# Malfoy/Brisk

Hardware: AMD Instinct MI355X
Metric: distinct k-mers indexed/sec (k=63,m=21) (higher is better)
Workload: dtype u64; 1 GPU; 1x MI355X: 50M synthetic 150 bp reads per GPU, k=63 m=21 b=14, uint8 counts, 15x coverage; reads_per_gpu=50000000, total_reads=50000000, part_bits=24, genome_len=500000000, parallelism=single GPU

## Files before the change

brisk_amd/csrc/brisk_capi.hip:

```cpp
#include "brisk_kernels.hip"

#include <algorithm>
#include <atomic>
#include <cerrno>
#include <chrono>
#include <cmath>
#include <cstdio>
#include <cstdlib>
#include <cstring>
#include <mutex>
#include <new>
#include <string>
#include <thread>
#include <vector>

#include <fcntl.h>
#include <sys/stat.h>
#include <unistd.h>

#include "../../include/brisk_hip.h"

#if !defined(__HIP_DEVICE_COMPILE__) && defined(__x86_64__)
#include <immintrin.h>
#define BRISK_HOST_AVX2 1
// ... 34 lines not shown
    u32 n_rerun, pad;
    unsigned long long kept;
    unsigned long long n_ovf;
    unsigned long long slice_sum;
    u32 upsert_done, pad2;
    struct Result { unsigned long long w[3]; } result;
    unsigned long long dbg_guard;
};
static_assert(sizeof(Counters::Scan) == sizeof(unsigned long long) + 2 * sizeof(u32) && sizeof(Counters::Touched) == 2 * sizeof(u32) + sizeof(unsigned long long), "ScanOut; k_touched, k_need");
static_assert(sizeof(Counters::Kmers) == 2 * sizeof(unsigned long long) && sizeof(Counters::Result) == 3 * sizeof(unsigned long long), "k_count_kmers: out[0..1]; k_checksum: out[0..2]");
static_assert(sizeof(Counters::Work) == 6 * sizeof(u32) && sizeof(Counters::Plan) == 2 * sizeof(u32), "32-bit counters throughout");
struct PinnedCounters : Counters {
    u32 n_huge;
    unsigned long long arena_used;
    unsigned long long n_rec_new;
    unsigned long long prof[3];
    unsigned long long answers;
};

}

struct brisk_hip_index {
    BriskParams P{};
    int device = 0;
    hipStream_t stream = nullptr;
    bool own_stream = false;
    std::string err;
    std::recursive_mutex call_mu;
    u64 n_parts = 0, n_buckets = 0;
    u64 max_batch_reads = 0;

    double* d_coef = nullptr;
    double* d_tabs = nullptr;
    ScanCfg scfg{};
    u32 dbg_touched_last = 0;
    u64 dbg_guard_last = 0;
    bool fresh = true;
    u32 insert_waves = 4096;
    u32 scan_waves = 0;
    size_t scan_lds = 0;
    bool scan_v1 = false;
    bool entry_ids = false;
    u32 count_mode = 0;
    bool use_vmm = false;
    bool scan_hist_valid = false;
    u64 arena_limit = 0;
    VmBuf vm_keys, vm_counts, vm_ids;
    unsigned long long* d_id_counter = nullptr;
    DevBuf seq_buf;
    u64 arena_cap = 0;
    u64 arena_used_host = 0;
    IndexDev ix{};
    DevBuf route_buf;
    DevBuf bins;
    DevBuf left;
    DevBuf huge;
    DevBuf pend;
    u64 n_pend = 0;
    bool pend_hist_ok = true;
    bool defer = true;
    bool verify = false;
    bool trace = false;
    DevBuf staging, parted, desc, chunk_buf, tags_a, tags_b, packed_tmp, bases_tmp, starts_tmp, sums_tmp, enum_out, lookup_buf;
    DevBuf packed_tmp2, starts_tmp2;
    DevBuf anchors, slot_buf, kout_tmp;
    DevBuf prof_out, prof_plan;
// ... 546 lines not shown
                HIPCHK(h, fetch_ctr_sync(h, &h->d_ctr->work));
                fprintf(stderr, "[brisk_hip] k_insert_first: %u of %u partitions taken in pairs, %u table-free, %u left over\n", h->h_ctr->work.n_pair, n_touched,
                        h->h_ctr->work.n_clean, h->h_ctr->work.n_left);
            }
        }
        if (n_huge) {
            if (sat) hipLaunchKernelGGL(k_insert_huge<true>, dim3(std::min<u32>(n_huge, 256u)), dim3(HG_THREADS), 0, h->stream, P, src, (const PartDesc*)h->desc.p,
                                        (const u32*)h->huge.p + 1, (const u32*)h->huge.p, h->ix);
            else hipLaunchKernelGGL(k_insert_huge<false>, dim3(std::min<u32>(n_huge, 256u)), dim3(HG_THREADS), 0, h->stream, P, src, (const PartDesc*)h->desc.p,
                                    (const u32*)h->huge.p + 1, (const u32*)h->huge.p, h->ix);
            if ((rc = launch_check(h, "k_insert_huge"))) return rc;
        }
    }
    h->nb_skmers += n_rec;
    h->dir_snapshot_valid = false;
    return BRISK_HIP_OK;
}

int launch_scan(brisk_hip_index* h, const u32* d_packed, const u64* d_starts, u64 n_items, const ScanOut& out, bool query_mode, bool plain,
                const ChunkCtl& cc, bool pos = false) {
    ProfScope ps(h, S_SCAN);
    if (plain && !pos) {
        BriskParams P = h->P;
        if (out.ret) {
            P.ext_bits -= P.cls_bits;
            P.cls_bits = 0;
        }
        hipLaunchKernelGGL(k_scan, dim3(nblocks(n_items, SCAN_BLOCK)), dim3(SCAN_BLOCK), 0, h->stream, P, d_packed, d_starts, n_items, h->d_coef,
                           out, query_mode ? 1 : 0);
    } else {
        const u32 bt = h->scan_waves * 64;
        const dim3 grid(nblocks(n_items, bt)), block(bt);
#define LAUNCH_SCAN2(NCH, MODE, KK, MM) \
    hipLaunchKernelGGL((k_scan2<NCH, MODE, KK, MM>), grid, block, h->scan_lds - scan_fixed_tabs(MM) * 8, h->stream, ScanArgs{h->P, h->scfg, d_packed, d_starts, n_items, h->d_tabs, out, cc})
#define LAUNCH_SCAN2_MODES(NCH, KK, MM)                    \
    {                                                      \
        if (pos && cc.vreads) LAUNCH_SCAN2(NCH, 4, KK, MM);  \
        else if (pos) LAUNCH_SCAN2(NCH, 3, KK, MM);        \
        else if (cc.vreads) LAUNCH_SCAN2(NCH, 2, KK, MM);  \
        else if (query_mode) LAUNCH_SCAN2(NCH, 1, KK, MM); \
        else LAUNCH_SCAN2(NCH, 0, KK, MM);                 \
    }
        const u32 k = h->P.k, m = h->P.m;
        if (k == 63 && m == 21) LAUNCH_SCAN2_MODES(0, 63, 21)
        else if (k == 31 && m == 15) LAUNCH_SCAN2_MODES(0, 31, 15)
        else if (k == 31 && m == 11) LAUNCH_SCAN2_MODES(0, 31, 11)
        else if (h->scfg.nch == 6) LAUNCH_SCAN2_MODES(6, 0, 0)
        else if (h->scfg.nch == 4) LAUNCH_SCAN2_MODES(4, 0, 0)
        else if (h->scfg.nch == 3) LAUNCH_SCAN2_MODES(3, 0, 0)
        else LAUNCH_SCAN2_MODES(0, 0, 0)
#undef LAUNCH_SCAN2_MODES
#undef LAUNCH_SCAN2
    }
    return launch_check(h, "k_scan");
}

enum class ScanMode { Insert, Query, Sequence, Position };
struct ScanReq {
    ScanMode mode;
    const u32* d_packed; const u64* d_starts; u64 n_reads;
    u64* d_rec; u64 cap;
    u64 kmer_bound = 0;
    bool with_hist = false, keep_hist = false;
    u32* d_tags = nullptr;
    u64* d_side = nullptr;
    const u64* d_slot_base = nullptr;
};
// ... 836 lines not shown
            return rc;
        }
    }
    if (h->profiling) {
        h->prof_ms[S_UPLOAD] += up_ms;
        h->prof_launches[S_UPLOAD] += subs.size();
    }
    return BRISK_HIP_OK;
}

int drain_profile(brisk_hip_index* h) {
    if (h->pending.empty()) return BRISK_HIP_OK;
    HIPCHK(h, hipStreamSynchronize(h->stream));
    for (auto& pe : h->pending) {
        float ms = 0;
        hipEventElapsedTime(&ms, pe.a, pe.b);
        h->prof_ms[pe.slot] += ms;
        h->prof_launches[pe.slot]++;
        hipEventDestroy(pe.a);
        hipEventDestroy(pe.b);
    }
    h->pending.clear();
    return BRISK_HIP_OK;
}

void free_all(brisk_hip_index* h) {
    hipStreamSynchronize(h->stream);
    auto fr = [](void* p) { if (p) hipFree(p); };
    for (DevBuf* b : {&h->huge, &h->left, &h->pend, &h->bins, &h->staging, &h->parted, &h->desc, &h->chunk_buf, &h->route_buf, &h->tags_a, &h->tags_b, &h->packed_tmp, &h->bases_tmp, &h->starts_tmp, &h->sums_tmp, &h->enum_out,
                      &h->lookup_buf, &h->packed_tmp2, &h->starts_tmp2, &h->anchors, &h->slot_buf, &h->kout_tmp, &h->prof_out, &h->prof_plan, &h->reck_buf, &h->ext_iv, &h->ext_tmp, &h->ext_src, &h->ink_mask, &h->ink_tmp, &h->ink_tab, &h->ink_raw, &h->ink_offs, &h->ink_packed, &h->pair_tab, &h->pair_iv, &h->pair_raw, &h->pair_fs, &h->split_off, &h->split_tab, &h->corr_sites, &h->corr_rows, &h->corr_cand, &h->corr_slots, &h->corr_tmp, &h->corr_tab})
        fr(b->p);
    fr(h->d_coef);
    fr(h->d_tabs);
    if (h->use_vmm) {
        pool_give(h->device, h->vm_keys, h->vm_counts, h->vm_ids);
    } else {
        fr(h->ix.keys);
        fr(h->ix.counts);
        fr(h->ix.ids);
    }
    fr(h->d_id_counter);
    fr(h->ix.err);
    fr(h->seq_buf.p);
    fr(h->ix.dir);
    fr(h->ix.cursor);
    fr(h->ix.bucket_bits);
    fr(h->ix.stats);
    fr(h->ix.slot_cur);
    fr(h->ix.slot_end);
    fr(h->d_hist);
    fr(h->d_ovf_cnt);
    fr(h->d_owner_cut);
    fr(h->d_off);
    fr(h->d_cur32);
    fr(h->d_touched);
    fr(h->d_block_sums);
    fr(h->d_ctr);
    if (h->h_ctr) hipHostFree(h->h_ctr);
    if (h->h_pin) hipHostFree(h->h_pin);
    for (auto& pe : h->pending) {
        hipEventDestroy(pe.a);
        hipEventDestroy(pe.b);
    }
    if (h->own_stream && h->stream) hipStreamDestroy(h->stream);
}

// ... 78 lines not shown
        HIPCHK(h, hipMalloc((void**)&h->d_coef, 128 * sizeof(double)));
        HIPCHK(h, hipMemsetAsync(h->d_coef, 0, 128 * sizeof(double), h->stream));
        HIPCHK(h, hipMemcpyAsync(h->d_coef, coef_table, 4 * m * sizeof(double), hipMemcpyHostToDevice, h->stream));
        {
            ScanCfg& c = h->scfg;
            c.nlow = std::min<u32>(32, k);
            c.nlow1 = std::min<u32>(32, k - 1);
            c.nch = cls_nch(m);
            c.qcap = 320;
            if (c.nch > CLS_MAX_CHUNKS) return fail(h, BRISK_HIP_EUNSUPPORTED, "minimizer too long for the class tables");
            const u32 n_tab = 128 + cls_base(m, c.nch);
            c.n_tab = n_tab;
            std::vector<double> tabs(n_tab, 0.0);
            for (u32 i = 0; i < 4u * m; i++) tabs[i] = coef_table[i];
            for (u32 ch = 0; ch < c.nch; ch++) {
                const u32 off = cls_off(m, ch), wd = cls_width(m, ch), base = cls_base(m, ch);
                c.chunk[ch] = (2 * off) | ((2 * wd) << 6) | (base << 10);
                for (u32 v = 0; v < (1u << (2 * wd)); v++) {
                    double a = 0.0, bsum = 0.0;
                    for (u32 i = off; i < off + wd; i++) {
                        const u32 nt = (v >> (2 * (i - off))) & 3;
                        if (i + 1 < m) a += coef_table[4 * (m - 1 - i) + nt];
                        if (i >= 1) bsum += coef_table[4 * (m - i) + nt];
                    }
                    const int64_t af = llround(std::ldexp(a, 24)), bf = llround(std::ldexp(bsum, 24));
                    u64 word = (u64)af + ((u64)bf << 32);
                    if (ch == 0) word += ((u64)CLS_BIAS << 32) + CLS_BIAS;
                    memcpy(&tabs[128 + base + v], &word, 8);
                }
            }
            HIPCHK(h, hipMalloc((void**)&h->d_tabs, n_tab * sizeof(double)));
            HIPCHK(h, hipMemcpyAsync(h->d_tabs, tabs.data(), n_tab * sizeof(double), hipMemcpyHostToDevice, h->stream));
            HIPCHK(h, hipStreamSynchronize(h->stream));
            const size_t fixed = (size_t)(n_tab + 9) * 8;
            const size_t lds_max = 160 * 1024;
            const bool spec = (k == 63 && m == 21) || (k == 31 && m == 15) || (k == 31 && m == 11);
            u32 blocks_per_cu = std::max<u32>(1, (u32)(scan_waves_per_eu(spec ? (int)k : 0, spec ? (int)m : 0) * 4) / 8);
            auto lds_of = [&](u32 q, u32 waves) { return fixed + waves * (size_t)(q + 96) * 8; };
            while (blocks_per_cu > 1 && blocks_per_cu * lds_of(224, 8) > lds_max - 2048) blocks_per_cu--;
            while (c.qcap > 224 && blocks_per_cu * lds_of(c.qcap, 8) > lds_max - 2048) c.qcap -= 32;
            if (const char* e = getenv("BRISK_SCAN_QCAP")) c.qcap = (u32)std::max(128, atoi(e));
            const size_t per_wave = (size_t)(c.qcap + 96) * 8;
            u32 wv = 8;
            if (lds_of(c.qcap, 8) > lds_max) wv = (u32)std::min<size_t>(16, (lds_max - fixed) / per_wave);
            if (const char* e = getenv("BRISK_SCAN_WAVES")) wv = (u32)std::min(16, std::max(1, atoi(e)));
            h->scan_waves = wv;
            h->scan_lds = fixed + wv * per_wave;
            static size_t lds_attr = 0;
            if (h->scan_lds > lds_attr) {
                lds_attr = h->scan_lds;
                struct FnLds { const void* fn; size_t fixed; };
#define SCAN2_FNS(NCH, KK, MM) FnLds{(const void*)k_scan2<NCH, 0, KK, MM>, scan_fixed_tabs(MM) * 8}, FnLds{(const void*)k_scan2<NCH, 1, KK, MM>, scan_fixed_tabs(MM) * 8}, \
                               FnLds{(const void*)k_scan2<NCH, 2, KK, MM>, scan_fixed_tabs(MM) * 8}, FnLds{(const void*)k_scan2<NCH, 3, KK, MM>, scan_fixed_tabs(MM) * 8}, \
                               FnLds{(const void*)k_scan2<NCH, 4, KK, MM>, scan_fixed_tabs(MM) * 8}
#define DEBUG_FN(NCH, MM) FnLds{(const void*)k_debug_keys<NCH, MM>, scan_fixed_tabs(MM) * 8}
                const FnLds fns[] = {SCAN2_FNS(0, 0, 0), SCAN2_FNS(3, 0, 0), SCAN2_FNS(4, 0, 0), SCAN2_FNS(6, 0, 0), SCAN2_FNS(0, 31, 11), SCAN2_FNS(0, 31, 15), SCAN2_FNS(0, 63, 21),
                                     DEBUG_FN(0, 0), DEBUG_FN(3, 0), DEBUG_FN(4, 0), DEBUG_FN(6, 0), DEBUG_FN(0, 11), DEBUG_FN(0, 15), DEBUG_FN(0, 21)};
#undef DEBUG_FN
#undef SCAN2_FNS
                for (const FnLds& f : fns) HIPCHK(h, hipFuncSetAttribute(f.fn, hipFuncAttributeMaxDynamicSharedMemorySize, (int)std::min(lds_attr, lds_max - f.fixed)));
            }
            const char* v1 = getenv("BRISK_SCAN_V1");
            h->scan_v1 = v1 && v1[0] == '1';
        }
        {
            const void* fns[] = {(const void*)k_insert<0, 0, 0>, (const void*)k_insert_big<0, 0, 0>, (const void*)k_insert_fast<3, 49, 4>, (const void*)k_insert_first<3, 49, 4>, (const void*)k_insert_fast<2, 17, 4>,
// ... 1770 lines not shown
    return launch_check(h, "k_synth");
}

BRISK_API int brisk_hip_debug_order_keys(brisk_hip_index* h, const uint64_t* mmers, uint64_t n, int exact, uint64_t* keys) {
    if (!h || (n && (!mmers || !keys))) return BRISK_HIP_EINVAL;
    if (!n) return BRISK_HIP_OK;
    HIPCHK(h, hipSetDevice(h->device));
    std::lock_guard<std::recursive_mutex> call_lock(h->call_mu);
    int rc;
    if ((rc = ensure(h, h->lookup_buf, n * 16))) return rc;
    u64* d_x = (u64*)h->lookup_buf.p;
    u64* d_k = d_x + n;
    HIPCHK(h, hipMemcpyAsync(d_x, mmers, n * 8, hipMemcpyHostToDevice, h->stream));
    const size_t lds = (size_t)h->scfg.n_tab * 8;
    HIPCHK(h, zero_ctr(h, &h->d_ctr->dbg_guard));
#define LAUNCH_DEBUG_KEYS(NCH, MM) \
    hipLaunchKernelGGL((k_debug_keys<NCH, MM>), dim3(nblocks(n, 256)), dim3(256), lds - scan_fixed_tabs(MM) * 8, h->stream, h->P, h->scfg, h->d_tabs, d_x, n, exact, d_k, &h->d_ctr->dbg_guard)
    const u32 k = h->P.k, m = h->P.m;
    if (k == 63 && m == 21) LAUNCH_DEBUG_KEYS(0, 21);
    else if (k == 31 && m == 15) LAUNCH_DEBUG_KEYS(0, 15);
    else if (k == 31 && m == 11) LAUNCH_DEBUG_KEYS(0, 11);
    else if (h->scfg.nch == 6) LAUNCH_DEBUG_KEYS(6, 0);
    else if (h->scfg.nch == 4) LAUNCH_DEBUG_KEYS(4, 0);
    else if (h->scfg.nch == 3) LAUNCH_DEBUG_KEYS(3, 0);
    else LAUNCH_DEBUG_KEYS(0, 0);
#undef LAUNCH_DEBUG_KEYS
    if ((rc = launch_check(h, "k_debug_keys"))) return rc;
    HIPCHK(h, hipMemcpyAsync(keys, d_k, n * 8, hipMemcpyDeviceToHost, h->stream));
    HIPCHK(h, fetch_ctr_sync(h, &h->d_ctr->dbg_guard));
    h->dbg_guard_last = h->h_ctr->dbg_guard;
    return BRISK_HIP_OK;
}

BRISK_API int brisk_hip_debug_guard_count(brisk_hip_index* h, uint64_t* n_guard) {
    if (!h || !n_guard) return BRISK_HIP_EINVAL;
    std::lock_guard<std::recursive_mutex> call_lock(h->call_mu);
    *n_guard = h->dbg_guard_last;
    return BRISK_HIP_OK;
}

BRISK_API int brisk_hip_debug_touched(brisk_hip_index* h, uint32_t* parts, uint64_t cap, uint64_t* n) {
    if (!h || !n || (cap && !parts)) return BRISK_HIP_EINVAL;
    HIPCHK(h, hipSetDevice(h->device));
    std::lock_guard<std::recursive_mutex> call_lock(h->call_mu);
    *n = h->dbg_touched_last;
    const u64 take = std::min<u64>(cap, h->dbg_touched_last);
    if (take) HIPCHK(h, hipMemcpyAsync(parts, h->d_touched, take * 4, hipMemcpyDeviceToHost, h->stream));
    HIPCHK(h, hipStreamSynchronize(h->stream));
    return BRISK_HIP_OK;
}

BRISK_API int brisk_hip_debug_directory(brisk_hip_index* h, const uint32_t* parts, uint64_t n, uint32_t* cnt, uint32_t* cap) {
    if (!h || (n && (!parts || !cnt || !cap))) return BRISK_HIP_EINVAL;
    HIPCHK(h, hipSetDevice(h->device));
    std::lock_guard<std::recursive_mutex> call_lock(h->call_mu);
    for (u64 i = 0; i < n; i++)
        if (parts[i] >= h->n_parts) return BRISK_HIP_EINVAL;
    std::vector<DirEnt> dir(h->n_parts);
    HIPCHK(h, hipMemcpyAsync(dir.data(), h->ix.dir, h->n_parts * sizeof(DirEnt), hipMemcpyDeviceToHost, h->stream));
    HIPCHK(h, hipStreamSynchronize(h->stream));
    for (u64 i = 0; i < n; i++) {
        cnt[i] = dir[parts[i]].cnt;
        cap[i] = dir[parts[i]].cap;
    }
    return BRISK_HIP_OK;
}
// ... 57 lines not shown
```

brisk_amd/csrc/brisk_scan.hip:

```cpp
__global__ void __launch_bounds__(256) k_pack_ascii(const uint8_t* __restrict__ bases, u64 n_bases, u32* __restrict__ packed, u64 n_words) {
    const u64 w = (u64)blockIdx.x * blockDim.x + threadIdx.x;
    if (w >= n_words) return;
    const u64 base = w * 16;
    u32 v = 0;
    if (base + 16 <= n_bases && ((uintptr_t)(bases + base) & 15) == 0) {
        const uint4 q = *reinterpret_cast<const uint4*>(bases + base);
        const u32 ws[4] = {q.x, q.y, q.z, q.w};
#pragma unroll
        for (int i = 0; i < 4; i++) {
#pragma unroll
            for (int j = 0; j < 4; j++) v = (v << 2) | ((ws[i] >> (8 * j + 1)) & 3u);
        }
    } else {
        for (int i = 0; i < 16; i++) {
            const u64 p = base + i;
            const u32 c = p < n_bases ? ((bases[p] >> 1) & 3u) : 0u;
            v = (v << 2) | c;
        }
    }
    packed[w] = v;
}

__device__ __forceinline__ u64 sm_mix(u64 z) {
    z = (z ^ (z >> 30)) * 0xBF58476D1CE4E5B9ull;
// ... 985 lines not shown
    if (!store) {
        q.meta |= MQ_TRUNC;
        return;
    }
    const u32 sh = 8 * keep;
    q.meta = (q.meta & ~((0xffu << sh) | (1u << (24 + keep)) | (1u << (27 + keep)) | MQ_TRUNC)) | ((step & 0xffu) << sh) | (rv ? 1u << (24 + keep) : 0u);
    if (keep == 0) q.k0 = h;
    if (keep <= 1) q.k1 = keep == 1 ? h : MQ_EMPTY;
    if (keep <= 2) q.k2 = keep == 2 ? h : MQ_EMPTY;
}
__device__ __forceinline__ void mq_pop_front(MinQueue& q) {
    q.k0 = q.k1;
    q.k1 = q.k2;
    q.k2 = MQ_EMPTY;
    q.meta = ((q.meta >> 8) & 0xffffu) | (((q.meta >> 25) & 3u) << 24) | (((q.meta >> 28) & 3u) << 27) | (q.meta & MQ_TRUNC);
}

#ifdef BRISK_PHASE_PROF
__device__ unsigned long long g_scan_cnt[8];
#define SCNT(i, v) scan_cnt[i] += (v);
#else
#define SCNT(i, v)
#endif

struct ScanArgs {
    BriskParams P;
    ScanCfg cfg;
    const u32* packed;
    const u64* starts;
    u64 n_reads;
    const double* g_tabs;
    ScanOut out;
    ChunkCtl cc;
};
struct ScanFlushArgs {
    BriskParams P;
    const u32* packed;
    ScanOut out;
    const u64* slot_base;
};
typedef const __attribute__((address_space(4))) u32* kernarg_words;
template <class T>
__device__ __forceinline__ T kernarg_field(kernarg_words ka, size_t off) {
    static_assert(sizeof(T) % 4 == 0 && alignof(T) <= 8, "whole dwords");
    struct Words {
        u32 w[sizeof(T) / 4];
    } v;
#pragma unroll
    for (u32 i = 0; i < sizeof(T) / 4; i++) v.w[i] = ka[off / 4 + i];
    return __builtin_bit_cast(T, v);
}
#ifndef SCAN_FLUSH_RELOAD
#define SCAN_FLUSH_RELOAD 1
#endif
template <int KK, int MM>
__device__ __forceinline__ ScanFlushArgs scan_flush_args(const ScanArgs& A) {
    ScanFlushArgs f;
#if !SCAN_FLUSH_RELOAD
    f.P = A.P;
    f.packed = A.packed;
    f.out = A.out;
    f.slot_base = A.cc.slot_base;
#else
    kernarg_words ka = (kernarg_words)__builtin_amdgcn_kernarg_segment_ptr();
    asm volatile("" : "+s"(ka));
    f.P = kernarg_field<BriskParams>(ka, offsetof(ScanArgs, P));
    f.packed = kernarg_field<const u32*>(ka, offsetof(ScanArgs, packed));
// ... 88 lines not shown
        hi_word = hw > 0xffffffffull ? 0xffffffffu : (u32)hw;
        for (int o = 32; o > 0; o >>= 1) hi_word = max(hi_word, (u32)__shfl_xor(hi_word, o, 64));
        if (lane == 0) s_wcnt[wid] = hi_word;
    }
    __syncthreads();
    if constexpr (ANCH) {
        for (u32 i = 0; i < (blockDim.x >> 6); i++) hi_word = max(hi_word, s_wcnt[i]);
        hi_word = __builtin_amdgcn_readfirstlane(hi_word);
        __syncthreads();
    }
    const bool live = len >= k;
    u32 nk = live ? (u32)(len - k + 1) : 0;
    u32 max_nk = nk;
    for (int o = 32; o > 0; o >>= 1) {
        const u32 y = __shfl_xor(max_nk, o, 64);
        max_nk = y > max_nk ? y : max_nk;
    }
#ifndef SCAN_UNIFORM_TRIP
#define SCAN_UNIFORM_TRIP 1
#endif
#if SCAN_UNIFORM_TRIP
    max_nk = (u32)__builtin_amdgcn_readfirstlane((int)max_nk);
#endif
    if (max_nk == 0) {
        const ScanFlushArgs fa = scan_flush_args<KK, MM>(A);
        scan_final_flush<CLS, POS, ANCH>(fa.P, fa.packed, fa.out, q_ent, s_q0, s_tag, 0, s_wcnt, s_wbase, fa.slot_base, hi_word);
        return;
    }
    const u64 KEY0 = order_key_fast<NCH, MM>(0, m, M, cfg, s_tabs, s_coef);
    const u64 KEY0s = read_lane_u64(KEY0, 0);

    u64 cr = 0, low64 = 0;
    if (live) low64 = load_nts(packed, q0 + (k - 1) - nlow1, nlow1);
    cr = rc64(low64 & M, m);

    u64 mini_hash;
    u32 mini_pos;
    bool reversed;
#ifndef SCAN_MINQUEUE
#define SCAN_MINQUEUE 1
#endif
#ifndef PROLOGUE_UNROLL
#define PROLOGUE_UNROLL 2
#endif
#define BRISK_PRAGMA_(x) _Pragma(#x)
#define BRISK_PRAGMA(x) BRISK_PRAGMA_(x)
    const bool mq_on = SCAN_MINQUEUE && (KK ? (KK <= 32) : (k <= 32));
    MinQueue mq{MQ_EMPTY, MQ_EMPTY, MQ_EMPTY, 0u};
    {
        const u32 Km = k - 1 - m;
        const u32 nwin = Km + 1 < nlow1 ? Km + 1 : nlow1;
        struct WinMin {
            u64 best;
            u32 first, last, flags;
        };
        auto pass = [&](auto exact_tag) -> WinMin {
            constexpr bool EXACT = decltype(exact_tag)::value;
            u64 best = ~0ull;
            u32 first = 0, last = 0, rf = 0, rl = 0;
            bool guard = false;
            u64 fw = low64 & M, rw = cr, above = low64 >> (2 * m);
            if (mq_on) mq = MinQueue{MQ_EMPTY, MQ_EMPTY, MQ_EMPTY, 0u};
#ifdef SCAN_ATTR_NOPROLOGUE
            for (u32 ii = 0; ii < 1; ii++) {
#else
            BRISK_PRAGMA(unroll PROLOGUE_UNROLL)
            for (u32 ii = 0; ii < nwin; ii++) {
#endif
                const u32 i = mq_on ? Km - ii : ii;
                u64 fwd, rcv;
                if (mq_on) {
                    fwd = (low64 >> (2 * i)) & M;
                    rcv = rc64(fwd, m);
                } else {
                    fwd = fw;
                    rcv = rw;
                    const u32 t = (u32)above & 3u;
                    above >>= 2;
                    fw = (fw >> 2) | ((u64)t << (2 * m - 2));
                    rw = ((rw << 2) & M) | (t ^ 2u);
                }
                const bool rv = rcv < fwd;
                const u64 x = rv ? rcv : fwd;
                u64 key;
                if (EXACT) key = order_key(x, m, M, s_coef);
                else {
#ifdef SCAN_ATTR_NOCLASS
                    key = order_key_fast<NCH, MM>(x, m, M, cfg, s_tabs, s_coef);
#else
                    key = ((u64)decy_class_guarded<NCH, MM>(x, cfg, s_tabs, guard) << 62) + mix2m(x, M);
#endif
                }
                const bool lt = key < best, eq = key == best;
                best = lt ? key : best;
                if (mq_on) {
                    first = lt || eq ? i : first;
                    rf = lt || eq ? (u32)rv : rf;
                    last = lt ? i : last;
                    rl = lt ? (u32)rv : rl;
                } else {
                    first = lt ? i : first;
                    rf = lt ? (u32)rv : rf;
                    last = lt || eq ? i : last;
                    rl = lt || eq ? (u32)rv : rl;
                }
                if (mq_on) mq_push(mq, key, 0u - 1u - i, rv);
            }
            return WinMin{best, first, last, rf | (rl << 1) | (guard ? 4u : 0u)};
        };
#ifdef SCAN_ATTR_PROLOGUE_TWICE
        if (__ballot(pass(std::false_type{}).flags & 4u) == 0x123456789ull) return;
        __builtin_amdgcn_s_barrier();
#endif
        WinMin wm = pass(std::false_type{});
        if (__ballot(wm.flags & 4u)) wm = pass(std::true_type{});
        u64 best = wm.best;
        u32 first = wm.first, last = wm.last;
        bool rf = wm.flags & 1u, rl = wm.flags & 2u;
        if (Km >= nwin) {
            if (KEY0 < best) {
                best = KEY0;
                first = nwin;
                last = Km;
                rf = rl = false;
            } else if (KEY0 == best) {
                last = Km;
                rl = false;
            }
        }
        u32 pos;
        bool rev, need_canon;
        resolve_ties(first, last, rf, rl, Km, false, false, &pos, &rev, &need_canon);
        if (need_canon && live) {
            const u64 hi = k - 1 > 32 ? load_nts(packed, q0, k - 1 - 32) : 0;
            if (!canonized_as_executed(mk128(low64, hi), k - 1)) rev = false;
        }
        mini_hash = best;
        mini_pos = pos;
        reversed = rev;
// ... 209 lines not shown
```

brisk_amd/hipapi.py:

```python
from __future__ import annotations

import atexit
import ctypes as C
import math
import os
import subprocess
import sys
import weakref
from typing import Optional, Sequence, Tuple

import numpy as np

HERE = os.path.dirname(os.path.abspath(__file__))
ROOT = os.path.dirname(HERE)
_LIB_NAME = os.environ.get("BRISK_HIP_LIB", "libbrisk_hip.so")

STATUS = {0: "OK", 1: "EINVAL", 2: "EUNSUPPORTED", 3: "EHIP", 4: "ENOMEM", 5: "ECAPACITY", 6: "ENODEVICE", 7: "EIO", 8: "EFORMAT"}
ECAPACITY = 5


class BriskHipError(RuntimeError):
    def __init__(self, code: int, msg: str = ""):
        self.code = code
        super().__init__(f"brisk_hip: {STATUS.get(code, code)} {msg}".strip())
# ... 54 lines not shown
                ("owner_rank", C.c_uint32), ("n_owners", C.c_uint32), ("arena_entries", C.c_uint64),
                ("max_batch_reads", C.c_uint64), ("entry_ids", C.c_uint32), ("immediate_inserts", C.c_uint32),
                ("count_mode", C.c_uint32)]


COUNT_MODES = {"wrap": 0, "saturate": 1}


class _Layout(C.Structure):
    _fields_ = [(n, C.c_uint32) for n in ("k", "m", "b", "m_reduc", "compacted_size", "allocated_bytes", "record_words",
                                          "part_bits", "n_owners", "owner_rank", "ext_bits", "cls_bits", "cls_width", "count_mode")]


class _SnapshotInfo(C.Structure):
    _fields_ = [(n, C.c_uint32) for n in ("struct_size", "version", "header_bytes", "k", "m", "b", "data_bytes", "part_bits", "ext_bits", "cls_bits",
                                          "cls_width", "key_words", "shift")] + \
               [(n, C.c_uint64) for n in ("n_entries", "n_partitions", "nb_skmers")] + [("checksum", C.c_uint64 * 3), ("n_blocks", C.c_uint64), ("file_bytes", C.c_uint64), ("count_mode", C.c_uint32)]


class _JointWindow(C.Structure):
    _fields_ = [(n, C.c_uint32) for n in ("min_self", "max_self", "min_other", "max_other", "keep_absent", "reserved")]


JOINT_ABSENT = 256
JOINT_STATES = 257

_u64p = np.ctypeslib.ndpointer(dtype=np.uint64, flags="C_CONTIGUOUS")
_u8p = np.ctypeslib.ndpointer(dtype=np.uint8, flags="C_CONTIGUOUS")

SYMBOLS = [
    "brisk_hip_abi_version", "brisk_hip_create", "brisk_hip_destroy", "brisk_hip_clear", "brisk_hip_last_error", "brisk_hip_sync",
    "brisk_hip_get_layout", "brisk_hip_insert_reads", "brisk_hip_insert_packed", "brisk_hip_get_reads", "brisk_hip_lookup",
    "brisk_hip_enumerate", "brisk_hip_stats", "brisk_hip_memory_info", "brisk_hip_insert_slack", "brisk_hip_reallocate", "brisk_hip_checksum", "brisk_hip_scan_packed", "brisk_hip_scan_bound", "brisk_hip_route_records",
    "brisk_hip_get_packed", "brisk_hip_get_kmers", "brisk_hip_get_kmers_packed", "brisk_hip_insert_records", "brisk_hip_set_owner_cuts", "brisk_hip_export_hist", "brisk_hip_export_hist_add", "brisk_hip_insert_records_hist", "brisk_hip_scan_query", "brisk_hip_route_tagged", "brisk_hip_query_records", "brisk_hip_pack_ascii", "brisk_hip_synth_reads", "brisk_hip_debug_order_keys", "brisk_hip_debug_guard_count", "brisk_hip_debug_touched", "brisk_hip_debug_directory", "brisk_hip_scan_sequence", "brisk_hip_upsert_kmers", "brisk_hip_find_kmers",
    "brisk_hip_enumerate_ids", "brisk_hip_count_spectrum", "brisk_hip_enumerate_range", "brisk_hip_prune",
    "brisk_hip_read_profile_reads", "brisk_hip_read_profile_packed",
    "brisk_hip_scan_kmers", "brisk_hip_record_kmers", "brisk_hip_answer_records", "brisk_hip_place_answers", "brisk_hip_profile_slots",
    "brisk_hip_select_intervals", "brisk_hip_extract_packed", "brisk_hip_trim_packed", "brisk_hip_trim_reads", "brisk_hip_unpack_ascii",
    "brisk_hip_intake_ascii", "brisk_hip_intake_reads", "brisk_hip_insert_raw_reads",
    "brisk_hip_fragment_intervals", "brisk_hip_pair_intervals", "brisk_hip_compose_intervals", "brisk_hip_extract_pairs_packed",
    "brisk_hip_trim_pairs_packed", "brisk_hip_trim_pairs_reads", "brisk_hip_clean_pairs_ascii", "brisk_hip_clean_pairs_reads",
    "brisk_hip_solid_runs", "brisk_hip_extract_fragments_packed", "brisk_hip_split_packed", "brisk_hip_split_reads",
    "brisk_hip_weak_sites", "brisk_hip_candidate_windows", "brisk_hip_decide_sites", "brisk_hip_apply_corrections", "brisk_hip_correct_packed", "brisk_hip_correct_reads",
    "brisk_hip_merge", "brisk_hip_intersect", "brisk_hip_subtract", "brisk_hip_compare", "brisk_hip_joint_spectrum", "brisk_hip_filter_joint", "brisk_hip_snapshot_info_read", "brisk_hip_save", "brisk_hip_load",
    "brisk_hip_profile_enable",
    "brisk_hip_profile_read", "brisk_hip_profile_reset",
]

_lib = None


def load() -> C.CDLL:
    global _lib
    if _lib is not None:
        return _lib
    path = library_path()
    if not os.path.exists(path):
        raise BriskHipError(6, f"{path} is missing: run __graft_entry__.build() (no CPU fallback exists)")
    L = C.CDLL(path)
    vp, u64, u32, i32 = C.c_void_p, C.c_uint64, C.c_uint32, C.c_int
    L.brisk_hip_abi_version.restype = u32
    L.brisk_hip_create.argtypes = [C.POINTER(vp), C.c_uint8, C.c_uint8, C.c_uint8, u32, C.POINTER(C.c_double), C.POINTER(_Options)]
    L.brisk_hip_destroy.argtypes = [vp]
    L.brisk_hip_clear.argtypes = [vp]
    L.brisk_hip_last_error.argtypes = [vp]
    L.brisk_hip_last_error.restype = C.c_char_p
    L.brisk_hip_sync.argtypes = [vp]
# ... 1096 lines not shown
        self._chk(self.L.brisk_hip_find_kmers(self.h, lo, hi, idx, len(lo), ids))
        return ids[: len(lo)]

    def enumerate_ids(self, chunk: int = 1 << 20):
        cur = C.c_uint64(0); n = C.c_uint64(0)
        out = [[], [], [], []]
        cap = chunk
        while True:
            lo = np.zeros(cap, np.uint64); hi = np.zeros(cap, np.uint64); idx = np.zeros(cap, np.uint8); ids = np.zeros(cap, np.uint32)
            rc = self.L.brisk_hip_enumerate_ids(self.h, C.byref(cur), lo, hi, idx, ids, cap, C.byref(n))
            if rc == ECAPACITY:
                cap *= 4
                continue
            self._chk(rc)
            if n.value == 0:
                break
            for a, v in zip(out, (lo, hi, idx, ids)):
                a.append(v[: n.value])
        dts = (np.uint64, np.uint64, np.uint8, np.uint32)
        return tuple(np.concatenate(a) if a else np.zeros(0, dt) for a, dt in zip(out, dts))

    def debug_order_keys(self, mmers, exact: bool = False) -> np.ndarray:
        x = np.ascontiguousarray(mmers, np.uint64)
        out = np.zeros(max(len(x), 1), np.uint64)
        self._chk(self.L.brisk_hip_debug_order_keys(self.h, x, len(x), 1 if exact else 0, out))
        return out[: len(x)]

    def debug_guard_count(self) -> int:
        n = C.c_uint64(0)
        self.L.brisk_hip_debug_guard_count.argtypes = [C.c_void_p, C.POINTER(C.c_uint64)]
        self._chk(self.L.brisk_hip_debug_guard_count(self.h, C.byref(n)))
        return int(n.value)

    def debug_touched(self) -> np.ndarray:
        f = self.L.brisk_hip_debug_touched
        f.argtypes = [C.c_void_p, C.c_void_p, C.c_uint64, C.POINTER(C.c_uint64)]
        n = C.c_uint64(0)
        self._chk(f(self.h, None, 0, C.byref(n)))
        out = np.zeros(max(int(n.value), 1), np.uint32)
        self._chk(f(self.h, out.ctypes.data, len(out), C.byref(n)))
        return out[: int(n.value)]

    def debug_directory(self, parts):
        f = self.L.brisk_hip_debug_directory
        f.argtypes = [C.c_void_p, C.c_void_p, C.c_uint64, C.c_void_p, C.c_void_p]
        p = np.ascontiguousarray(parts, np.uint32)
        cnt, cap = np.zeros(max(len(p), 1), np.uint32), np.zeros(max(len(p), 1), np.uint32)
        self._chk(f(self.h, p.ctypes.data, len(p), cnt.ctypes.data, cap.ctypes.data))
        return cnt[: len(p)], cap[: len(p)]

    def profile_enable(self, on: bool = True):
        self._chk(self.L.brisk_hip_profile_enable(self.h, 1 if on else 0))

    def profile_reset(self):
        self._chk(self.L.brisk_hip_profile_reset(self.h))

    def profile_read(self) -> dict:
        n = C.c_uint32()
        names = (C.c_char_p * 16)()
        launches = (C.c_uint64 * 16)()
        ms = (C.c_double * 16)()
        self._chk(self.L.brisk_hip_profile_read(self.h, C.byref(n), names, launches, ms))
        return {names[i].decode(): {"launches": launches[i], "ms": ms[i]} for i in range(n.value)}
```

include/brisk_hip.h:

```cpp
#ifndef BRISK_HIP_H
#define BRISK_HIP_H

#include <stddef.h>
#include <stdint.h>

#ifdef __cplusplus
extern "C" {
#endif

#define BRISK_HIP_ABI_VERSION 4

enum {
    BRISK_HIP_OK = 0,
    BRISK_HIP_EINVAL = 1,
    BRISK_HIP_EUNSUPPORTED = 2,
    BRISK_HIP_EHIP = 3,
    BRISK_HIP_ENOMEM = 4,
    BRISK_HIP_ECAPACITY = 5,
    BRISK_HIP_ENODEVICE = 6,
    BRISK_HIP_EIO = 7,
    BRISK_HIP_EFORMAT = 8
};

typedef struct brisk_hip_index brisk_hip_index;
// ... 294 lines not shown
                           uint64_t *d_out, uint32_t *d_tags_out, uint64_t *counts);
int brisk_hip_query_records(brisk_hip_index *h, const uint64_t *d_records, uint64_t n_records, uint64_t *d_sums);

int brisk_hip_scan_kmers(brisk_hip_index *h, const uint32_t *d_packed, const uint64_t *d_starts, uint64_t n_reads,
                         uint64_t *d_records, uint32_t *d_tags, uint64_t *d_anchors, uint64_t cap_records,
                         uint64_t *n_records, uint64_t *n_slots);
int brisk_hip_record_kmers(brisk_hip_index *h, const uint64_t *d_records, uint64_t n_records, uint64_t *d_offsets);
int brisk_hip_answer_records(brisk_hip_index *h, const uint64_t *d_records, uint64_t n_records, const uint64_t *d_offsets,
                             uint16_t *d_answers);
int brisk_hip_place_answers(brisk_hip_index *h, const uint64_t *d_records, const uint32_t *d_tags, const uint64_t *d_anchors,
                            uint64_t n_records, const uint64_t *d_offsets, const uint16_t *d_answers,
                            uint16_t *d_slots, uint64_t n_slots);
int brisk_hip_profile_slots(brisk_hip_index *h, const uint16_t *d_slots, const uint64_t *d_starts, uint64_t n_reads,
                            uint32_t solid_min, brisk_hip_read_profile *d_out);

int brisk_hip_scan_sequence(brisk_hip_index *h, const char *bases, uint64_t len, uint64_t cap_kmers,
                            uint64_t *skm_ret, uint32_t *skm_n, uint64_t *km_lo, uint64_t *km_hi, uint8_t *km_idx,
                            uint64_t *n_skm);
int brisk_hip_upsert_kmers(brisk_hip_index *h, const uint64_t *kmer_lo, const uint64_t *kmer_hi, const uint8_t *minimizer_idx,
                           uint64_t n, uint32_t *ids, uint8_t *newly);
int brisk_hip_find_kmers(brisk_hip_index *h, const uint64_t *kmer_lo, const uint64_t *kmer_hi, const uint8_t *minimizer_idx,
                         uint64_t n, uint32_t *ids);
int brisk_hip_enumerate_ids(brisk_hip_index *h, uint64_t *cursor, uint64_t *out_lo, uint64_t *out_hi,
                            uint8_t *out_minimizer_idx, uint32_t *out_ids, uint64_t cap, uint64_t *n_out);

int brisk_hip_pack_ascii(brisk_hip_index *h, const char *d_bases, uint64_t n_bases, uint32_t *d_packed);
int brisk_hip_unpack_ascii(brisk_hip_index *h, const uint32_t *d_packed, uint64_t first_nt, uint64_t n_nts, char *d_bases);
int brisk_hip_synth_reads(brisk_hip_index *h, uint64_t genome_len, uint64_t first_read, uint64_t n_reads,
                          uint32_t read_len, uint64_t seed_g, uint64_t seed_r,
                          uint32_t *d_packed, uint64_t *d_starts);

int brisk_hip_debug_order_keys(brisk_hip_index *h, const uint64_t *mmers, uint64_t n, int exact, uint64_t *keys);
int brisk_hip_debug_guard_count(brisk_hip_index *h, uint64_t *n_guard);
int brisk_hip_debug_touched(brisk_hip_index *h, uint32_t *parts, uint64_t cap, uint64_t *n);
int brisk_hip_debug_directory(brisk_hip_index *h, const uint32_t *parts, uint64_t n, uint32_t *cnt, uint32_t *cap);

#define BRISK_HIP_PROFILE_SLOTS 16
int brisk_hip_profile_enable(brisk_hip_index *h, int on);
int brisk_hip_profile_read(brisk_hip_index *h, uint32_t *n_slots, const char **names, uint64_t *launches, double *ms);
int brisk_hip_profile_reset(brisk_hip_index *h);

#ifdef __cplusplus
}
#endif
#endif
```

Before: 35.91 billion k-mers/s.

## Precompute minimizer results for the last window prefix via lookup table

Adds a device table, indexed by the trailing 10 nucleotides (4^10 entries) and filled once at setup, that stores each entry's minimum order key, the first and last positions of that minimum, and strand flags for the final m-mer windows. When k=63 and m=21, the scan prologue evaluates PFX fewer windows itself and merges the stored result with one global load. This removes order-key hashing work from the prologue. In exchange it adds a random 8 MB table gather per item, and correctness depends on the table windows matching the unmasked windows in the scan. A debug API is added so the table contents can be inspected.

```diff
diff --git a/brisk_amd/csrc/brisk_capi.hip b/brisk_amd/csrc/brisk_capi.hip
--- a/brisk_amd/csrc/brisk_capi.hip
+++ b/brisk_amd/csrc/brisk_capi.hip
@@ -90,6 +90,8 @@
 
     double* d_coef = nullptr;
     double* d_tabs = nullptr;
+    u64* d_prefix_tab = nullptr;
+    u32 prefix_nts = 0;
     ScanCfg scfg{};
     u32 dbg_touched_last = 0;
     u64 dbg_guard_last = 0;
@@ -702,7 +704,7 @@
         const u32 bt = h->scan_waves * 64;
         const dim3 grid(nblocks(n_items, bt)), block(bt);
 #define LAUNCH_SCAN2(NCH, MODE, KK, MM) \
-    hipLaunchKernelGGL((k_scan2<NCH, MODE, KK, MM>), grid, block, h->scan_lds - scan_fixed_tabs(MM) * 8, h->stream, ScanArgs{h->P, h->scfg, d_packed, d_starts, n_items, h->d_tabs, out, cc})
+    hipLaunchKernelGGL((k_scan2<NCH, MODE, KK, MM>), grid, block, h->scan_lds - scan_fixed_tabs(MM) * 8, h->stream, ScanArgs{h->P, h->scfg, d_packed, d_starts, n_items, h->d_tabs, out, cc, h->d_prefix_tab})
 #define LAUNCH_SCAN2_MODES(NCH, KK, MM)                    \
     {                                                      \
         if (pos && cc.vreads) LAUNCH_SCAN2(NCH, 4, KK, MM);  \
@@ -1605,6 +1607,7 @@
         fr(b->p);
     fr(h->d_coef);
     fr(h->d_tabs);
+    fr(h->d_prefix_tab);
     if (h->use_vmm) {
         pool_give(h->device, h->vm_keys, h->vm_counts, h->vm_ids);
     } else {
@@ -1749,6 +1752,13 @@
             HIPCHK(h, hipMalloc((void**)&h->d_tabs, n_tab * sizeof(double)));
             HIPCHK(h, hipMemcpyAsync(h->d_tabs, tabs.data(), n_tab * sizeof(double), hipMemcpyHostToDevice, h->stream));
             HIPCHK(h, hipStreamSynchronize(h->stream));
+            if ((h->prefix_nts = scan_prefix_nts((int)k, (int)m))) {
+                const u64 n_ent = 1ull << (2 * h->prefix_nts);
+                HIPCHK(h, hipMalloc((void**)&h->d_prefix_tab, n_ent * 8));
+                hipLaunchKernelGGL(k_prefix_table_fill<21>, dim3(nblocks(n_ent, 256)), dim3(256), 0, h->stream, h->d_tabs, h->prefix_nts, h->d_prefix_tab);
+                int rc = launch_check(h, "k_prefix_table_fill");
+                if (rc) return rc;
+            }
             const size_t fixed = (size_t)(n_tab + 9) * 8;
             const size_t lds_max = 160 * 1024;
             const bool spec = (k == 63 && m == 21) || (k == 31 && m == 15) || (k == 31 && m == 11);
@@ -3585,6 +3595,19 @@
     return BRISK_HIP_OK;
 }
 
+BRISK_API int brisk_hip_debug_prefix_table(brisk_hip_index* h, uint64_t first, uint64_t n, uint64_t* out) {
+    if (!h || (n && !out)) return BRISK_HIP_EINVAL;
+    std::lock_guard<std::recursive_mutex> call_lock(h->call_mu);
+    if (!h->d_prefix_tab) return fail(h, BRISK_HIP_EUNSUPPORTED, "this geometry's scan has no prefix table");
+    const u64 n_ent = 1ull << (2 * h->prefix_nts);
+    if (first > n_ent || n > n_ent - first) return BRISK_HIP_EINVAL;
+    if (!n) return BRISK_HIP_OK;
+    HIPCHK(h, hipSetDevice(h->device));
+    HIPCHK(h, hipMemcpyAsync(out, h->d_prefix_tab + first, n * 8, hipMemcpyDeviceToHost, h->stream));
+    HIPCHK(h, hipStreamSynchronize(h->stream));
+    return BRISK_HIP_OK;
+}
+
 BRISK_API int brisk_hip_debug_guard_count(brisk_hip_index* h, uint64_t* n_guard) {
     if (!h || !n_guard) return BRISK_HIP_EINVAL;
     std::lock_guard<std::recursive_mutex> call_lock(h->call_mu);
diff --git a/brisk_amd/csrc/brisk_scan.hip b/brisk_amd/csrc/brisk_scan.hip
--- a/brisk_amd/csrc/brisk_scan.hip
+++ b/brisk_amd/csrc/brisk_scan.hip
@@ -1041,7 +1041,45 @@
     const double* g_tabs;
     ScanOut out;
     ChunkCtl cc;
+    const u64* prefix_tab;
 };
+
+#ifndef SCAN_PREFIX_TABLE
+#define SCAN_PREFIX_TABLE 1
+#endif
+#ifndef SCAN_PREFIX_NTS
+#define SCAN_PREFIX_NTS 10
+#endif
+__host__ __device__ constexpr u32 scan_prefix_nts(int KK, int MM) { return SCAN_PREFIX_TABLE && KK == 63 && MM == 21 ? (u32)SCAN_PREFIX_NTS : 0u; }
+static_assert(SCAN_PREFIX_NTS >= 1 && SCAN_PREFIX_NTS <= 14, "window offsets take four bits, and 4^T entries have to be worth their memory");
+static_assert(scan_prefix_nts(63, 21) <= 21 && 2 * 21 + 2 <= 44, "the table's windows are unmasked ones, and class and mix fit below the window fields");
+#define PFX_FIRST 44
+#define PFX_LAST 48
+#define PFX_RF 52
+#define PFX_RL 53
+template <int MM>
+__global__ void __launch_bounds__(256) k_prefix_table_fill(const double* __restrict__ g_tabs, u32 T, u64* __restrict__ tab) {
+    __shared__ double s_coef[128];
+    if (threadIdx.x < 128) s_coef[threadIdx.x] = g_tabs[threadIdx.x];
+    __syncthreads();
+    const u64 t = (u64)blockIdx.x * blockDim.x + threadIdx.x;
+    if (t >= (1ull << (2 * T))) return;
+    constexpr u64 M = (1ull << (2 * MM)) - 1;
+    u64 best = ~0ull;
+    u32 first = 0, last = 0, rf = 0, rl = 0;
+    for (u32 j = 0; j < T; j++) {
+        const u64 fwd = t >> (2 * j), rcv = rc64(fwd, MM);
+        const bool rv = rcv < fwd;
+        const u64 key = order_key(rv ? rcv : fwd, MM, M, s_coef);
+        const bool lt = key < best, eq = key == best;
+        best = lt ? key : best;
+        first = lt ? j : first;
+        rf = lt ? (u32)rv : rf;
+        last = lt || eq ? j : last;
+        rl = lt || eq ? (u32)rv : rl;
+    }
+    tab[t] = (best & M) | ((best >> 62) << (2 * MM)) | ((u64)first << PFX_FIRST) | ((u64)last << PFX_LAST) | ((u64)rf << PFX_RF) | ((u64)rl << PFX_RL);
+}
 struct ScanFlushArgs {
     BriskParams P;
     const u32* packed;
@@ -1196,6 +1234,9 @@
 
     u64 cr = 0, low64 = 0;
     if (live) low64 = load_nts(packed, q0 + (k - 1) - nlow1, nlow1);
+    constexpr u32 PFX = scan_prefix_nts(KK, MM);
+    u64 pfx_entry = 0;
+    if constexpr (PFX > 0) pfx_entry = A.prefix_tab[low64 >> (64 - 2 * PFX)];
     cr = rc64(low64 & M, m);
 
     u64 mini_hash;
@@ -1229,7 +1270,7 @@
             for (u32 ii = 0; ii < 1; ii++) {
 #else
             BRISK_PRAGMA(unroll PROLOGUE_UNROLL)
-            for (u32 ii = 0; ii < nwin; ii++) {
+            for (u32 ii = 0; ii < nwin - PFX; ii++) {
 #endif
                 const u32 i = mq_on ? Km - ii : ii;
                 u64 fwd, rcv;
@@ -1269,6 +1310,15 @@
                     rl = lt || eq ? (u32)rv : rl;
                 }
                 if (mq_on) mq_push(mq, key, 0u - 1u - i, rv);
+            }
+            if constexpr (PFX > 0) {
+                const u64 key = (pfx_entry & M) | ((pfx_entry >> (2 * MM)) << 62);
+                const bool lt = key < best, le = key <= best;
+                best = lt ? key : best;
+                first = lt ? (nwin - PFX) + ((u32)(pfx_entry >> PFX_FIRST) & 15u) : first;
+                rf = lt ? (u32)(pfx_entry >> PFX_RF) & 1u : rf;
+                last = le ? (nwin - PFX) + ((u32)(pfx_entry >> PFX_LAST) & 15u) : last;
+                rl = le ? (u32)(pfx_entry >> PFX_RL) & 1u : rl;
             }
             return WinMin{best, first, last, rf | (rl << 1) | (guard ? 4u : 0u)};
         };
diff --git a/brisk_amd/hipapi.py b/brisk_amd/hipapi.py
--- a/brisk_amd/hipapi.py
+++ b/brisk_amd/hipapi.py
@@ -110,7 +110,7 @@
     "brisk_hip_abi_version", "brisk_hip_create", "brisk_hip_destroy", "brisk_hip_clear", "brisk_hip_last_error", "brisk_hip_sync",
     "brisk_hip_get_layout", "brisk_hip_insert_reads", "brisk_hip_insert_packed", "brisk_hip_get_reads", "brisk_hip_lookup",
     "brisk_hip_enumerate", "brisk_hip_stats", "brisk_hip_memory_info", "brisk_hip_insert_slack", "brisk_hip_reallocate", "brisk_hip_checksum", "brisk_hip_scan_packed", "brisk_hip_scan_bound", "brisk_hip_route_records",
-    "brisk_hip_get_packed", "brisk_hip_get_kmers", "brisk_hip_get_kmers_packed", "brisk_hip_insert_records", "brisk_hip_set_owner_cuts", "brisk_hip_export_hist", "brisk_hip_export_hist_add", "brisk_hip_insert_records_hist", "brisk_hip_scan_query", "brisk_hip_route_tagged", "brisk_hip_query_records", "brisk_hip_pack_ascii", "brisk_hip_synth_reads", "brisk_hip_debug_order_keys", "brisk_hip_debug_guard_count", "brisk_hip_debug_touched", "brisk_hip_debug_directory", "brisk_hip_scan_sequence", "brisk_hip_upsert_kmers", "brisk_hip_find_kmers",
+    "brisk_hip_get_packed", "brisk_hip_get_kmers", "brisk_hip_get_kmers_packed", "brisk_hip_insert_records", "brisk_hip_set_owner_cuts", "brisk_hip_export_hist", "brisk_hip_export_hist_add", "brisk_hip_insert_records_hist", "brisk_hip_scan_query", "brisk_hip_route_tagged", "brisk_hip_query_records", "brisk_hip_pack_ascii", "brisk_hip_synth_reads", "brisk_hip_debug_order_keys", "brisk_hip_debug_guard_count", "brisk_hip_debug_prefix_table", "brisk_hip_debug_touched", "brisk_hip_debug_directory", "brisk_hip_scan_sequence", "brisk_hip_upsert_kmers", "brisk_hip_find_kmers",
     "brisk_hip_enumerate_ids", "brisk_hip_count_spectrum", "brisk_hip_enumerate_range", "brisk_hip_prune",
     "brisk_hip_read_profile_reads", "brisk_hip_read_profile_packed",
     "brisk_hip_scan_kmers", "brisk_hip_record_kmers", "brisk_hip_answer_records", "brisk_hip_place_answers", "brisk_hip_profile_slots",
@@ -1273,6 +1273,13 @@
         self._chk(self.L.brisk_hip_debug_guard_count(self.h, C.byref(n)))
         return int(n.value)
 
+    def debug_prefix_table(self, first: int, n: int) -> np.ndarray:
+        f = self.L.brisk_hip_debug_prefix_table
+        f.argtypes = [C.c_void_p, C.c_uint64, C.c_uint64, C.c_void_p]
+        out = np.zeros(max(int(n), 1), np.uint64)
+        self._chk(f(self.h, first, n, out.ctypes.data))
+        return out[: int(n)]
+
     def debug_touched(self) -> np.ndarray:
         f = self.L.brisk_hip_debug_touched
         f.argtypes = [C.c_void_p, C.c_void_p, C.c_uint64, C.POINTER(C.c_uint64)]
diff --git a/include/brisk_hip.h b/include/brisk_hip.h
--- a/include/brisk_hip.h
+++ b/include/brisk_hip.h
@@ -350,6 +350,7 @@
 
 int brisk_hip_debug_order_keys(brisk_hip_index *h, const uint64_t *mmers, uint64_t n, int exact, uint64_t *keys);
 int brisk_hip_debug_guard_count(brisk_hip_index *h, uint64_t *n_guard);
+int brisk_hip_debug_prefix_table(brisk_hip_index *h, uint64_t first, uint64_t n, uint64_t *out);
 int brisk_hip_debug_touched(brisk_hip_index *h, uint32_t *parts, uint64_t cap, uint64_t *n);
 int brisk_hip_debug_directory(brisk_hip_index *h, const uint32_t *parts, uint64_t n, uint32_t *cnt, uint32_t *cap);
 
```

Measured after the change: 36.26 billion k-mers/s, median of 6. About the same (+1.0%).
